# andrewdalpino/UltraZoom

Measured on AMD Instinct MI355X. Metric: upscaled MPix/sec, MewZoom-4X 1080p bf16 batched inference, higher is better.
Workload: dtype bf16; 1 GPU; MewZoom-4X 96ch/40L bf16, 16 x 1080x1920 -> 4320x7680 per GPU; global_batch=16, parallelism=batch-sharded x1, images_in_flight=0

## Files before the change

### ultrazoom_amd/csrc/mz_mix16.h

```cpp
#pragma once
#include "mz_device.h"

namespace mz {

__device__ __forceinline__ void mix_blend_pair(float& o0, float& o1, const float b0, const float b1, const float x0, const float x1,
                                               const float z0, const float z1, const float inv_s) {
    float d0, d1;
    asm("v_mul_f32 %0, 0xbfb8aa3b, %4\n\t"
        "v_mul_f32 %1, 0xbfb8aa3b, %5\n\t"
        "v_exp_f32 %0, %0\n\t"
        "v_exp_f32 %1, %1\n\t"
        "v_fma_f32 %0, %0, %10, %10\n\t"
        "v_fma_f32 %1, %1, %10, %10\n\t"
        "v_rcp_f32 %0, %0\n\t"
        "v_rcp_f32 %1, %1\n\t"
        "v_sub_f32 %2, %8, %6\n\t"
        "v_sub_f32 %3, %9, %7\n\t"
        "v_fma_f32 %0, %0, %2, %6\n\t"
        "v_fma_f32 %1, %1, %3, %7"
        : "=&v"(o0), "=&v"(o1), "=&v"(d0), "=&v"(d1)
        : "v"(b0), "v"(b1), "v"(x0), "v"(x1), "v"(z0), "v"(z1), "s"(inv_s));
}

struct MixFrag {
    u32x4 w[3][2];
};
template <class TT, int G>
__device__ __forceinline__ void mix16_group(f32x4 (&acc)[2][12], MixFrag& f, const u32x4 (&xb)[2], uint32_t b_addr) {
    constexpr int n = G % 6, wp = G % 3;
    if constexpr (G + 2 < 24) {
        f.w[(G + 2) % 3][0] = lds_read128<(((G + 2) / 6) * 12 + 2 * ((G + 2) % 6)) * 1024>(b_addr);
        f.w[(G + 2) % 3][1] = lds_read128<(((G + 2) / 6) * 12 + 2 * ((G + 2) % 6) + 1) * 1024>(b_addr);
    }
    __builtin_amdgcn_sched_barrier(0);
    constexpr int p0 = G & 1, p1 = p0 ^ 1;
    mma16<TT>(acc[p0][2 * n], f.w[wp][0], xb[p0]);
    mma16<TT>(acc[p0][2 * n + 1], f.w[wp][1], xb[p0]);
    mma16<TT>(acc[p1][2 * n + 1], f.w[wp][1], xb[p1]);
    mma16<TT>(acc[p1][2 * n], f.w[wp][0], xb[p1]);
    __builtin_amdgcn_sched_barrier(0);
    if constexpr (G + 1 < 24) wait_w16<(G + 2 < 24 ? 2 : 0)>(f.w[(G + 1) % 3][0], f.w[(G + 1) % 3][1]);
}
template <class TT, int KS> __device__ __forceinline__ void mix16_kstep(f32x4 (&acc)[2][12], MixFrag& f, const u32x4 (&xb)[2], uint32_t b_addr) {
    mix16_group<TT, KS * 6 + 0>(acc, f, xb, b_addr);
    mix16_group<TT, KS * 6 + 1>(acc, f, xb, b_addr);
    mix16_group<TT, KS * 6 + 2>(acc, f, xb, b_addr);
    mix16_group<TT, KS * 6 + 3>(acc, f, xb, b_addr);
    mix16_group<TT, KS * 6 + 4>(acc, f, xb, b_addr);
    mix16_group<TT, KS * 6 + 5>(acc, f, xb, b_addr);
}

template <class TT>
__global__ __launch_bounds__(576) void mix16_kernel(const ConvArgs a) {
    constexpr int STAGE = 4 * 12 * 1024;
    extern __shared__ __attribute__((aligned(16))) char smem[];
    const int tid = threadIdx.x;
    const int lane = tid & 63;
    const int w = __builtin_amdgcn_readfirstlane(tid >> 6);
    int mtile, ntile;
    if (!map_tile(a, mtile, ntile)) return;
    const int nsteps = a.nchunks16;
    const int nstages = nsteps >> 2;

    if (w == 8) {
        const char* src = (const char*)a.wpk16 + (size_t)ntile * nsteps * (12 * 1024) + lane * 16;
        auto issue = [&](int st) __attribute__((always_inline)) {
            char* dst = smem + (st & 1) * STAGE;
#pragma unroll
            for (int j = 0; j < 48; ++j) glds16(src + (size_t)st * STAGE + j * 1024, dst + j * 1024);
        };
        issue(0);
        for (int st = 0; st < nstages; ++st) {
            wait_vmcnt<0>();
            __builtin_amdgcn_s_barrier();
            if (st + 1 < nstages) issue(st + 1);
        }
        return;
    }

    const int g = lane >> 4, c = lane & 15;
    const long long hw = (long long)a.Ho * a.Wo;
    const long long M = (long long)a.B * hw;
    const int half_steps = nsteps >> 1;
    const uint32_t tensor_bytes = (uint32_t)((long long)a.B * a.p0 * hw * 16);
    const __amdgpu_buffer_rsrc_t xr = __builtin_amdgcn_make_buffer_rsrc((void*)a.in0, 0, (int)tensor_bytes, 0x00020000);
    const __amdgpu_buffer_rsrc_t zr = __builtin_amdgcn_make_buffer_rsrc((void*)a.in1, 0, (int)tensor_bytes, 0x00020000);
    uint32_t voff[2];
    uint32_t vpix[2];
#pragma unroll
    for (int pf = 0; pf < 2; ++pf) {
        const long long m = (long long)mtile * 256 + 32 * w + 16 * pf + c;
        const bool in = m < M;
        const long long mm = in ? m : 0;
        const int bimg = (int)(mm / hw);
        const long long pix = mm - (long long)bimg * hw;
        vpix[pf] = in ? (uint32_t)((((long long)bimg * a.p0) * hw + pix) * 16) : 0xffffffffu;
        voff[pf] = in ? (uint32_t)((((long long)bimg * a.p0 + g) * hw + pix) * 16) : 0xffffffffu;
    }
    const uint32_t step_bytes = (uint32_t)(4 * hw * 16);
    auto load_b = [&](int ks, u32x4 (&xb)[2]) __attribute__((always_inline)) {
        const bool isz = ks >= half_steps;
        const int kk = ks >= nsteps ? 0 : (isz ? ks - half_steps : ks);
        const int so = __builtin_amdgcn_readfirstlane((int)(kk * step_bytes));
#pragma unroll
        for (int pf = 0; pf < 2; ++pf)
            xb[pf] = isz ? __builtin_amdgcn_raw_buffer_load_b128(zr, (int)voff[pf], so, 0)
                         : __builtin_amdgcn_raw_buffer_load_b128(xr, (int)voff[pf], so, 0);
    };
    f32x4 acc[2][12];
#pragma unroll
    for (int pf = 0; pf < 2; ++pf)
#pragma unroll
        for (int nf = 0; nf < 12; ++nf) acc[pf][nf] = f32x4{0.f, 0.f, 0.f, 0.f};
    const uint32_t lds_base = (uint32_t)(uintptr_t)(__attribute__((address_space(3))) char*)smem;
    const uint32_t b_lane = lds_base + lane * 16;
    u32x4 xb0[2], xb1[2], xb2[2];
    load_b(0, xb0);
    load_b(1, xb1);
    MixFrag f;
    auto stage_head = [&](uint32_t b_addr) __attribute__((always_inline)) {
        __builtin_amdgcn_s_barrier();
        f.w[0][0] = lds_read128<0>(b_addr);
        f.w[0][1] = lds_read128<1024>(b_addr);
        f.w[1][0] = lds_read128<2048>(b_addr);
        f.w[1][1] = lds_read128<3072>(b_addr);
        wait_w16<2>(f.w[0][0], f.w[0][1]);
    };
    for (int st = 0; st < nstages; st += 3) {
        const int ks = 4 * st;
        uint32_t b_addr = b_lane + (st & 1) * STAGE;
        stage_head(b_addr);
        load_b(ks + 2, xb2);  mix16_kstep<TT, 0>(acc, f, xb0, b_addr);
        load_b(ks + 3, xb0);  mix16_kstep<TT, 1>(acc, f, xb1, b_addr);
        load_b(ks + 4, xb1);  mix16_kstep<TT, 2>(acc, f, xb2, b_addr);
        load_b(ks + 5, xb2);  mix16_kstep<TT, 3>(acc, f, xb0, b_addr);
        b_addr = b_lane + ((st + 1) & 1) * STAGE;
        stage_head(b_addr);
        load_b(ks + 6, xb0);  mix16_kstep<TT, 0>(acc, f, xb1, b_addr);
        load_b(ks + 7, xb1);  mix16_kstep<TT, 1>(acc, f, xb2, b_addr);
        load_b(ks + 8, xb2);  mix16_kstep<TT, 2>(acc, f, xb0, b_addr);
        load_b(ks + 9, xb0);  mix16_kstep<TT, 3>(acc, f, xb1, b_addr);
        b_addr = b_lane + (st & 1) * STAGE;
        stage_head(b_addr);
        load_b(ks + 10, xb1); mix16_kstep<TT, 0>(acc, f, xb2, b_addr);
        load_b(ks + 11, xb2); mix16_kstep<TT, 1>(acc, f, xb0, b_addr);
        load_b(ks + 12, xb0); mix16_kstep<TT, 2>(acc, f, xb1, b_addr);
        load_b(ks + 13, xb1); mix16_kstep<TT, 3>(acc, f, xb2, b_addr);
    }
    const int nbase = ntile * 192;
    const uint32_t plane_bytes = (uint32_t)(hw * 16);
    typedef uint32_t u32x2_ __attribute__((ext_vector_type(2)));
    struct XZ { u32x2_ x[2], z[2]; };
    auto request = [&](int i, XZ& q) __attribute__((always_inline)) {
        const int pf = i / 6, n = i - 6 * pf;
        const bool in = vpix[pf] != 0xffffffffu;
#pragma unroll
        for (int k = 0; k < 2; ++k) {
            const int nf = 2 * n + k;
            const int plane = (nbase >> 3) + 2 * nf + (g >> 1);
            const uint32_t off = in ? vpix[pf] + (uint32_t)plane * plane_bytes + (g & 1) * 8 : 0xffffffffu;
            q.x[k] = __builtin_amdgcn_raw_buffer_load_b64(xr, (int)off, 0, 0);
            q.z[k] = __builtin_amdgcn_raw_buffer_load_b64(zr, (int)off, 0, 0);
        }
    };
    auto finish = [&](int i, const XZ& q) __attribute__((always_inline)) {
        const int pf = i / 6, n = i - 6 * pf;
        const bool in = vpix[pf] != 0xffffffffu;
        float v[8];
#pragma unroll
        for (int k = 0; k < 2; ++k) {
            const int nf = 2 * n + k;
            float xv[4], zv[4];
            unpack2<TT>(q.x[k][0], xv[0], xv[1]); unpack2<TT>(q.x[k][1], xv[2], xv[3]);
            unpack2<TT>(q.z[k][0], zv[0], zv[1]); unpack2<TT>(q.z[k][1], zv[2], zv[3]);
            float o0, o1, o2, o3;
            mix_blend_pair(o0, o1, acc[pf][nf][0], acc[pf][nf][1], xv[0], xv[1], zv[0], zv[1], a.inv_mix_scale);
            mix_blend_pair(o2, o3, acc[pf][nf][2], acc[pf][nf][3], xv[2], xv[3], zv[2], zv[3], a.inv_mix_scale);
            acc[pf][nf] = f32x4{o0, o1, o2, o3};
        }
#pragma unroll
        for (int j = 0; j < 4; ++j) {
            const float ea = acc[pf][2 * n][j], eb = acc[pf][2 * n + 1][j];
            const auto sw = __builtin_amdgcn_permlane16_swap(__builtin_bit_cast(uint32_t, ea), __builtin_bit_cast(uint32_t, eb), false, false);
            const uint32_t s0 = sw[0], s1 = sw[1];
            v[j] = __builtin_bit_cast(float, s0);
            v[4 + j] = __builtin_bit_cast(float, s1);
        }
        const int cu = 2 * (2 * n + (g & 1)) + (g >> 1);
        if (in) st_unit<TT>((char*)a.out + vpix[pf] + (long long)((nbase >> 3) + cu) * plane_bytes, v);
    };
    XZ qa, qb;
    request(0, qa);
#pragma unroll
    for (int i = 0; i < 12; i += 2) {
        request(i + 1, qb);
        __builtin_amdgcn_sched_barrier(0);
        finish(i, qa);
        if (i + 2 < 12) request(i + 2, qa);
        __builtin_amdgcn_sched_barrier(0);
        finish(i + 1, qb);
    }
}

template <class TT>
__global__ __launch_bounds__(512) void mix16b_kernel(const ConvArgs a) {
    constexpr int STAGE = 4 * 12 * 1024;
    extern __shared__ __attribute__((aligned(16))) char smem[];
    const int tid = threadIdx.x;
    const int lane = tid & 63;
    const int w = __builtin_amdgcn_readfirstlane(tid >> 6);
    {
        const char* wsrc = (const char*)a.wpk16 + lane * 16 + w * (18 * 1024);
        char* dst = smem + w * (18 * 1024);
#pragma unroll
        for (int j = 0; j < 18; ++j) glds16(wsrc + j * 1024, dst + j * 1024);
    }
    const int g = lane >> 4, c = lane & 15;
    const long long hw = (long long)a.Ho * a.Wo;
    const long long M = (long long)a.B * hw;
    const uint32_t tensor_bytes = (uint32_t)((long long)a.B * a.p0 * hw * 16);
    const __amdgpu_buffer_rsrc_t xr = __builtin_amdgcn_make_buffer_rsrc((void*)a.in0, 0, (int)tensor_bytes, 0x00020000);
    const __amdgpu_buffer_rsrc_t zr = __builtin_amdgcn_make_buffer_rsrc((void*)a.in1, 0, (int)tensor_bytes, 0x00020000);
    const __amdgpu_buffer_rsrc_t orr = __builtin_amdgcn_make_buffer_rsrc((void*)a.out, 0, (int)tensor_bytes, 0x00020000);
    const uint32_t step_bytes = (uint32_t)(4 * hw * 16);
    const float inv_hw = 1.0f / (float)hw;
    const int hwi = (int)hw, Mi = (int)M;
    auto offsets = [&](int u, uint32_t (&vo)[2]) __attribute__((always_inline)) {
#pragma unroll
        for (int pf = 0; pf < 2; ++pf) {
            const int m = u * 32 + 16 * pf + c;
            const bool in = m < Mi;
            const int mm = in ? m : 0;
            int bimg = (int)((float)mm * inv_hw);
            int pix = mm - bimg * hwi;
            if (pix < 0) { bimg -= 1; pix += hwi; }
            if (pix >= hwi) { bimg += 1; pix -= hwi; }
            vo[pf] = in ? ((uint32_t)(bimg * a.p0 + g) * (uint32_t)hwi + (uint32_t)pix) * 16u : 0xffffffffu;
        }
    };
    const int nunits = (Mi + 31) / 32;
    const int stride = (int)gridDim.x * 8;
    int u = (int)blockIdx.x * 8 + w;
    uint32_t voff[2];
    offsets(u, voff);
    u32x4 R[12][2];
#pragma unroll
    for (int i = 0; i < 6; ++i) {
        const int so = __builtin_amdgcn_readfirstlane((int)(i * step_bytes));
#pragma unroll
        for (int pf = 0; pf < 2; ++pf) R[i][pf] = __builtin_amdgcn_raw_buffer_load_b128(xr, (int)voff[pf], so, 0);
    }
#pragma unroll
    for (int i = 0; i < 6; ++i) {
        const int so = __builtin_amdgcn_readfirstlane((int)(i * step_bytes));
#pragma unroll
        for (int pf = 0; pf < 2; ++pf) R[6 + i][pf] = __builtin_amdgcn_raw_buffer_load_b128(zr, (int)voff[pf], so, 0);
    }
    __builtin_amdgcn_sched_barrier(0);
    wait_vmcnt<0>();
    __builtin_amdgcn_s_barrier();
    const uint32_t lds_base = (uint32_t)(uintptr_t)(__attribute__((address_space(3))) char*)smem;
    const uint32_t b_lane = lds_base + lane * 16;
    MixFrag f;
    auto stage_head = [&](uint32_t b_addr) __attribute__((always_inline)) {
        f.w[0][0] = lds_read128<0>(b_addr);
        f.w[0][1] = lds_read128<1024>(b_addr);
        f.w[1][0] = lds_read128<2048>(b_addr);
        f.w[1][1] = lds_read128<3072>(b_addr);
        wait_w16<2>(f.w[0][0], f.w[0][1]);
    };
    while (u < nunits) {
        const int un = u + stride;
        uint32_t vnext[2];
        offsets(un, vnext);
        __builtin_amdgcn_sched_barrier(0);
        f32x4 acc[2][12];
#pragma unroll
        for (int pf = 0; pf < 2; ++pf)
#pragma unroll
            for (int nf = 0; nf < 12; ++nf) acc[pf][nf] = f32x4{0.f, 0.f, 0.f, 0.f};
        stage_head(b_lane);
        mix16_kstep<TT, 0>(acc, f, R[0], b_lane);
        mix16_kstep<TT, 1>(acc, f, R[1], b_lane);
        mix16_kstep<TT, 2>(acc, f, R[2], b_lane);
        mix16_kstep<TT, 3>(acc, f, R[3], b_lane);
        stage_head(b_lane + STAGE);
        mix16_kstep<TT, 0>(acc, f, R[4], b_lane + STAGE);
        mix16_kstep<TT, 1>(acc, f, R[5], b_lane + STAGE);
        mix16_kstep<TT, 2>(acc, f, R[6], b_lane + STAGE);
        mix16_kstep<TT, 3>(acc, f, R[7], b_lane + STAGE);
        stage_head(b_lane + 2 * STAGE);
        mix16_kstep<TT, 0>(acc, f, R[8], b_lane + 2 * STAGE);
        mix16_kstep<TT, 1>(acc, f, R[9], b_lane + 2 * STAGE);
        mix16_kstep<TT, 2>(acc, f, R[10], b_lane + 2 * STAGE);
        mix16_kstep<TT, 3>(acc, f, R[11], b_lane + 2 * STAGE);
#pragma unroll
        for (int m = 0; m < 6; ++m) {
            const int so = __builtin_amdgcn_readfirstlane((int)(m * step_bytes));
#pragma unroll
            for (int pf = 0; pf < 2; ++pf) {
                float v[8];
#pragma unroll
                for (int q = 0; q < 4; ++q) {
                    float xl, xh, zl, zh;
                    unpack2<TT>(R[m][pf][q], xl, xh);
                    unpack2<TT>(R[6 + m][pf][q], zl, zh);
                    mix_blend_pair(v[2 * q], v[2 * q + 1], acc[pf][2 * m + (q >> 1)][2 * (q & 1)], acc[pf][2 * m + (q >> 1)][2 * (q & 1) + 1], xl, xh, zl, zh,
                                   a.inv_mix_scale);
                }
                u32x4 t;
                if constexpr (TT::IS_BF16) {
                    t[0] = pack_bf16(v[0], v[1]); t[1] = pack_bf16(v[2], v[3]); t[2] = pack_bf16(v[4], v[5]); t[3] = pack_bf16(v[6], v[7]);
                } else {
                    t[0] = pack_f16(v[0], v[1]); t[1] = pack_f16(v[2], v[3]); t[2] = pack_f16(v[4], v[5]); t[3] = pack_f16(v[6], v[7]);
                }
                store16_soff(t, orr, (int)voff[pf], so);
            }
#pragma unroll
            for (int pf = 0; pf < 2; ++pf) {
                R[m][pf] = __builtin_amdgcn_raw_buffer_load_b128(xr, (int)vnext[pf], so, 0);
                R[6 + m][pf] = __builtin_amdgcn_raw_buffer_load_b128(zr, (int)vnext[pf], so, 0);
            }
            __builtin_amdgcn_sched_barrier(0);
        }
        u = un;
        voff[0] = vnext[0];
        voff[1] = vnext[1];
    }
}

}
```

### ultrazoom_amd/csrc/mz_mix16.hip

```cpp
#include "mz_mix16.h"

namespace mz {

hipError_t launch_mix16(int dtype, const ConvArgs& a, hipStream_t s) {
    if (!walk_ok(a)) return hipErrorInvalidValue;
    if (a.nchunks16 <= 0 || a.nchunks16 % 12) return hipErrorInvalidValue;
    const size_t lds = 2 * 4 * 12 * 1024;
    switch (dtype) {
        case DT_BF16: return launch_lds<mix16_kernel<TBF16>>(a.grid, 576, lds, a, s);
        case DT_F16: return launch_lds<mix16_kernel<TF16>>(a.grid, 576, lds, a, s);
        default: return hipErrorInvalidValue;
    }
}

hipError_t launch_mix16b(int dtype, const ConvArgs& a, hipStream_t s, int workgroups) {
    if (a.mtiles <= 0 || a.ntiles != 1 || workgroups <= 0) return hipErrorInvalidValue;
    if (a.nchunks16 != 12) return hipErrorInvalidValue;
    const size_t lds = 3 * 4 * 12 * 1024;
    const int grid = a.mtiles < workgroups ? a.mtiles : workgroups;
    switch (dtype) {
        case DT_BF16: return launch_lds<mix16b_kernel<TBF16>>(grid, 512, lds, a, s);
        case DT_F16: return launch_lds<mix16b_kernel<TF16>>(grid, 512, lds, a, s);
        default: return hipErrorInvalidValue;
    }
}

}
```

### ultrazoom_amd/csrc/mz_runner.h

```cpp
#pragma once
#include <cmath>
#include <cstring>
#include <map>
#include <utility>

#include "mz_err.h"
#include "mz_select.h"

namespace mz {

struct DevBuf {
    void* p = nullptr;
    DevBuf() = default;
    DevBuf(DevBuf&& o) noexcept : p(o.p) { o.p = nullptr; }
    ~DevBuf() {
        if (p) (void)hipFree(p);
    }
    hipError_t alloc(size_t bytes) { return p ? hipSuccess : hipMalloc(&p, bytes); }
};

struct ConvW : LayerPlan {
    DevBuf packed[PK_COUNT];
};
using BlockW = Block<ConvW>;
inline const ConvW& weights(const LayerPlan* c) { return *static_cast<const ConvW*>(c); }

inline int pack_conv(ConvW& c, int dtype, const float* w_dev, hipStream_t s) {
    for (int l = 0; l < PK_COUNT; ++l) {
        if (!c.has(l)) continue;
        HIPCHK(c.packed[l].alloc(pack_bytes(c, l)));
        HIPCHK(launch_pack(pack_args(c, l, dtype, w_dev, c.packed[l].p), s));
    }
    return MZ_OK;
}

struct ProfRec {
    hipEvent_t a, b;
    double flops, bytes;
    int kind, B, H, W, cin, cout, nt, ntiles, mtiles, n_fast;
};

struct LaunchCtx {
    DevBuf zero_page;
    Knobs knobs = read_knobs();
    std::map<std::vector<int>, std::pair<DevBuf, int>> tile_tabs;
    bool prof = false;
    std::vector<ProfRec> recs;
    size_t recs_used = 0;
    int init(hipStream_t s) {
        HIPCHK(zero_page.alloc(4096));
        HIPCHK(hipMemsetAsync(zero_page.p, 0, 4096, s));
        return MZ_OK;
    }
    ~LaunchCtx() {
        for (auto& r : recs) {
            (void)hipEventDestroy(r.a);
            (void)hipEventDestroy(r.b);
        }
    }
};

inline unsigned long long* debug_buffer() {
    static unsigned long long* buf = nullptr;
    static bool tried = false;
    if (!tried) {
        tried = true;
        if (getenv("MZ_DEBUG_STAMPS")) {
            if (hipMalloc((void**)&buf, 16 * 64 * 8 * sizeof(unsigned long long)) != hipSuccess) buf = nullptr;
            else (void)hipMemset(buf, 0, 16 * 64 * 8 * sizeof(unsigned long long));
        }
    }
    return buf;
}

inline float inv_sigmoid(float alpha) {
    const float v = 1.0f + std::exp(-alpha);
    return std::isfinite(v) ? v : 3.402823466e+38f;
}

struct Runner {
    LaunchCtx& ctx;
    hipStream_t s;
    int dtype;
    int rc = MZ_OK;
    const Knobs knobs = ctx.knobs;
    int io_u8 = 0;
    int cus = std::max(0, device_cus());

    ProfRec* prof_begin(int kind, const ConvArgs& a, const LayerPlan& c, double flops, double bytes) {
        if (!ctx.prof) return nullptr;
        if (ctx.recs_used == ctx.recs.size()) {
            ProfRec n;
            if (hipEventCreate(&n.a) != hipSuccess || hipEventCreate(&n.b) != hipSuccess) return nullptr;
            ctx.recs.push_back(n);
        }
        ProfRec* r = &ctx.recs[ctx.recs_used++];
        r->flops = flops; r->bytes = bytes;
        r->kind = kind; r->B = a.B; r->H = a.H; r->W = a.W; r->cin = c.cin; r->cout = c.cout; r->nt = c.nt; r->ntiles = a.ntiles;
        r->mtiles = a.mtiles; r->n_fast = a.gm * 1000 + a.gn;
        (void)hipEventRecord(r->a, s);
        return r;
    }

    int check(hipError_t e, const char* what) {
        if (e != hipSuccess && rc == MZ_OK) rc = hip_rc(e, what);
        return rc;
    }

    void base_args(ConvArgs& a, const ConvW& c, const void* in0, void* out, int B, int H, int W, int cp_out, const Walk& w) {
        memset(&a, 0, sizeof(a));
        a.wpk = c.packed[PK_MAIN].p;
        a.zero = ctx.zero_page.p;
        a.dbg = debug_buffer();
        a.nchunks = c.nchunks;
        a.nchunks_real = c.nchunks_real;
        a.in0 = in0; a.out = out;
        a.B = B; a.H = H; a.W = W; a.Ho = H; a.Wo = W;
        a.p0 = c.cp0 * dtype_size(dtype) / 16;
        a.cp_out = cp_out;
        a.p_out = a.cp_out * dtype_size(dtype) / 16;
        put_walk(a, w);
    }

    void tile_table(ConvArgs& a, const Walk& w, int th, int tw, int wgs) {
        const int pad = 4 * ((wgs > 256 ? wgs : 256) / 8) + 8;
        const std::vector<int> key = {th, tw, a.B, w.tiles_x, w.tiles_y, w.ntiles, w.gm, w.gn, w.grid, w.blk4, pad};
        auto it = ctx.tile_tabs.find(key);
        if (it == ctx.tile_tabs.end()) {
            std::vector<uint32_t> t;
            t.reserve(2 * ((size_t)w.mtiles * w.ntiles + pad));
            tile_list(w, th, tw, t);
            const int n = (int)(t.size() / 2);
            t.resize(t.size() + 2 * (size_t)pad, 0u);
            DevBuf d;
            if (check(d.alloc(t.size() * 4), "tile table")) return;
            if (check(hipMemcpy(d.p, t.data(), t.size() * 4, hipMemcpyHostToDevice), "tile table upload")) return;
            it = ctx.tile_tabs.emplace(key, std::make_pair(std::move(d), n)).first;
        }
        a.tile_tab = it->second.first.p;
        a.grid = it->second.second;
    }

    hipError_t launch_kernel(const KernelChoice& ch, const ConvArgs& a, int nt) {
        switch (ch.kernel) {
            case K_CONV256: return launch_conv256(dtype, ch.mode, nt, a, s);
            case K_CONV3W: return launch_conv3w(dtype, ch.mode, nt, a, s);
            case K_CONV3P: return launch_conv3p(dtype, ch.mode, nt, a, s);
            case K_CONV3S: return launch_conv3s(dtype, ch.mode, nt, a, s);
            case K_CONV3R: return launch_conv3r(dtype, a, s);
            case K_CONV3T: return launch_conv3t(dtype, a, s);
            case K_MIX16: return launch_mix16(dtype, a, s);
            case K_MIX16B: return launch_mix16b(dtype, a, s, ch.persist);
        }
        return hipErrorInvalidValue;
    }
    void launch(const KernelChoice& ch, const ConvArgs& a, int nt, ProfRec* r, const char* what = nullptr) {
        if (!what) what = g_last_kernel = kernel_name(ch);
        check(launch_kernel(ch, a, nt), what);
        if (r) (void)hipEventRecord(r->b, s);
    }

    void conv3(const Conv3Call& k) {
        if (rc) return;
        const KernelChoice ch = choose_conv3(knobs, dtype, k, cus);
        if (!ch.ok) { rc = fail(MZ_ERR_INVALID_ARGUMENT, "%s", ch.why); return; }
        const ConvW& c = weights(k.c);
        const int B = k.B, H = k.H, W = k.W;
        const double sz = dtype_size(dtype);
        const double px = (double)B * H * W;
        const int tiles_x = (W + ch.tw - 1) / ch.tw, tiles_y = (H + ch.th - 1) / ch.th;
        const Walk w = pick_order(tiles_x, tiles_y, B * tiles_x * tiles_y, c.ntiles, (double)pack_bytes(c, PK_MAIN), px * c.cp0 * sz, knobs);
        ConvArgs a;
        base_args(a, c, k.in, k.out, B, H, W, k.epi == EPI_D2S ? c.cq_p : pad16(c.cout), w);
        a.src = SRC_PLAIN;
        a.epi = k.epi; a.silu = k.silu;
        a.Hout = k.Hout; a.Wout = k.Wout;
        a.img = k.img; a.R = k.R; a.clamp = k.clamp;
        if (k.epi == EPI_FINAL) { a.Hi = k.Hout / k.R; a.Wi = k.Wout / k.R; a.io_u8 = io_u8; }
        if (k.epi == EPI_FINAL && k.views) {
            a.view = 1;
            for (int i = 0; i < 4; ++i) { a.vin[i] = k.views->in[i]; a.vout[i] = k.views->out[i]; }
            a.win_y0 = k.views->y0; a.win_x0 = k.views->x0; a.win_h = k.views->h; a.win_w = k.views->w;
        }
        const bool fused = ch.fused;
        if (fused) {
            a.in1 = k.xin;
            a.p1 = pad16(c.cout) * dtype_size(dtype) / 16;
            a.wmix = weights(k.mixf).packed[PK_MAIN].p;
            a.mix_pieces = k.mixf->nchunks * k.mixf->nt;
            const int slot = ch.mode == MODE_C3W16 ? stage_bytes<MODE_C3W16>(c.nt) : stage_bytes<MODE_C3W8>(c.nt);
            const int ncx = a.p1 / 2;
            a.x_via_lds = (a.mix_pieces * 1024 + 8 * ncx * 1024 <= 2 * slot) ? 1 : 0;
            a.mix_scale = 1.0f / (1.0f + std::exp(-k.alpha));
            a.inv_mix_scale = inv_sigmoid(k.alpha);
        }
        a.geo = ch.geo;
        a.ragged_planes = ch.ragged_planes;
        if (ch.layout != PK_MAIN) {
            a.wpk16 = c.packed[ch.layout].p;
            a.nchunks16 = pack_shape(c, ch.layout).nchunks;
            if (fused) a.wmix16 = weights(k.mixf).packed[ch.gate].p;
        }
        if (ch.tile_list) tile_table(a, w, ch.th, ch.tw, ch.persist);
        if (rc) return;
        a.persist = std::min((a.grid + 7) / 8 * 8, ch.persist);
        a.film_gamma = k.gamma; a.film_beta = k.beta;
        const double flops = 2.0 * px * 9.0 * c.cin * c.cout + (fused ? 2.0 * px * 2.0 * c.cout * c.cout : 0.0);
        const double bytes = px * (c.cin + c.cout) * sz + 9.0 * c.cin * c.cout * sz + (fused ? px * c.cout * sz : 0.0);
        launch(ch, a, c.nt, prof_begin(0, a, c, flops, bytes));
    }

    void mix(const ConvW& c, float alpha, const void* x, const void* z, void* out, int B, int H, int W) {
        if (rc) return;
        const KernelChoice ch = choose_mix(knobs, dtype, c, B, H, W, cus);
        const int sz = dtype_size(dtype);
        const long long npix = (long long)B * H * W;
        const bool mix16 = ch.layout != PK_MAIN;
        const PackShape sh = pack_shape(c, ch.layout);
        ConvArgs a;
        base_args(a, c, x, out, B, H, W, pad16(c.cout),
                  pick_order(0, 0, (int)((npix + 255) / 256), sh.ntiles, (double)pack_bytes(c, PK_MAIN),
                             (double)npix * (c.cp0 + pad16(c.c1)) * sz, knobs, mix16 ? 32 : 64));
        a.in1 = z; a.p1 = pad16(c.c1) * sz / 16;
        a.nchunks0 = c.cp0 / chunk_channels(dtype);
        a.src = SRC_CONCAT;
        a.epi = EPI_MIX;
        a.mix_scale = 1.0f / (1.0f + std::exp(-alpha));
        a.inv_mix_scale = inv_sigmoid(alpha);
        if (mix16) {
            a.wpk16 = c.packed[ch.layout].p;
            a.nchunks16 = sh.nchunks;
        }
        launch(ch, a, c.nt, prof_begin(1, a, c, 2.0 * (double)npix * c.cin * c.cout, (double)npix * 3.0 * c.cout * sz));
    }

    void crush(const ConvW& c, const void* in, void* out, int B, int H, int W) {
        if (rc) return;
        const double sz = dtype_size(dtype);
        const long long npix = (long long)B * (H / 2) * (W / 2);
        ConvArgs a;
        base_args(a, c, in, out, B, H, W, pad16(c.cout),
                  pick_order(0, 0, (int)((npix + 255) / 256), c.ntiles, (double)pack_bytes(c, PK_MAIN), (double)B * H * W * c.cp0 * sz, knobs, 64));
        a.Ho = H / 2; a.Wo = W / 2;
        a.nchunks0 = c.cp0 / chunk_channels(dtype);
        a.src = SRC_CRUSH;
        a.epi = EPI_STORE;
        ProfRec* r = prof_begin(2, a, c, 2.0 * (double)npix * 4.0 * c.cin * c.cout, ((double)B * H * W * c.cin + (double)npix * c.cout) * sz);
        KernelChoice ch;
        ch.ok = true; ch.kernel = K_CONV256; ch.mode = MODE_GEMM1;
        launch(ch, a, c.nt, r, "crush launch");
    }
};

}
```

### ultrazoom_amd/csrc/mz_select.h

```cpp
#pragma once
#include <math.h>

#include <vector>

#include "mz_plan.h"
#include "mz_view_check.h"

namespace mz {

struct Walk {
    int tiles_x = 0, tiles_y = 0;
    int mtiles = 0, ntiles = 0;
    int gm = 1, gn = 1, groups_m = 0, grid = 0;
    int blk4 = 0;
    float inv_gsz = 1.f, inv_groups_m = 1.f, inv_gn = 1.f, inv_tpi = 1.f, inv_tiles_x = 1.f, inv_bsz = 1.f;
};

inline Walk group_walk(int tiles_x, int tiles_y, int mtiles, int ntiles, int gm, int gn, int blk4) {
    Walk w;
    w.tiles_x = tiles_x; w.tiles_y = tiles_y; w.mtiles = mtiles; w.ntiles = ntiles;
    w.gm = gm; w.gn = gn; w.blk4 = blk4;
    w.groups_m = (mtiles + gm - 1) / gm;
    w.grid = (int)((long long)w.groups_m * ((ntiles + gn - 1) / gn) * gm * gn);
    w.inv_gsz = 1.0f / (float)(gm * gn);
    w.inv_groups_m = 1.0f / (float)w.groups_m;
    w.inv_gn = 1.0f / (float)gn;
    if (tiles_x > 0) {
        w.inv_tpi = 1.0f / (float)(tiles_x * tiles_y);
        w.inv_tiles_x = 1.0f / (float)tiles_x;
        w.inv_bsz = 1.0f / (float)(4 * tiles_x);
    }
    return w;
}

inline Walk pick_order(int tiles_x, int tiles_y, int mtiles, int ntiles, double weight_bytes, double act_bytes, const Knobs& k,
                       int resident_per_xcd = 32) {
    int best_gm = mtiles, best_gn = 1;
    double best = 1e300;
    for (int gn = 1; gn <= ntiles; ++gn) {
        if (gn > resident_per_xcd) break;
        if (ntiles % gn != 0 && gn != ntiles) continue;
        int gm = resident_per_xcd / gn;
        if (gm < 1) gm = 1;
        if (gm > mtiles) gm = mtiles;
        const double groups_n = ceil((double)ntiles / gn), groups_m = ceil((double)mtiles / gm);
        const double traffic = act_bytes * groups_n + weight_bytes * groups_m;
        if (traffic < best) { best = traffic; best_gm = gm; best_gn = gn; }
    }
    return group_walk(tiles_x, tiles_y, mtiles, ntiles, best_gm, best_gn, k.blk4 && tiles_x > 0 && 4 * tiles_x < 65536 ? 1 : 0);
}

inline void put_walk(ConvArgs& a, const Walk& w) {
    a.tiles_x = w.tiles_x; a.tiles_y = w.tiles_y; a.mtiles = w.mtiles; a.ntiles = w.ntiles;
    a.gm = w.gm; a.gn = w.gn; a.groups_m = w.groups_m; a.grid = w.grid; a.blk4 = w.blk4;
    a.inv_gsz = w.inv_gsz; a.inv_groups_m = w.inv_groups_m; a.inv_gn = w.inv_gn;
    a.inv_tpi = w.inv_tpi; a.inv_tiles_x = w.inv_tiles_x; a.inv_bsz = w.inv_bsz;
}

inline void tile_list(const Walk& a, int th, int tw, std::vector<uint32_t>& t) {
    const int tpi = a.tiles_x * a.tiles_y, gsz = a.gm * a.gn;
    for (int L = 0; L < a.grid; ++L) {
        const int group = L / gsz, within = L % gsz;
        const int gi_n = group / a.groups_m, gi_m = group % a.groups_m;
        const int mt = gi_m * a.gm + within / a.gn, nt = gi_n * a.gn + within % a.gn;
        if (mt >= a.mtiles || nt >= a.ntiles) continue;
        const int b = mt / tpi, trem = mt % tpi;
        int tyi, txi;
        if (!a.blk4) {
            tyi = trem / a.tiles_x; txi = trem % a.tiles_x;
        } else {
            const int bsz = 4 * a.tiles_x, br = trem / bsz, rem = trem % bsz;
            const int rows = std::min(4, a.tiles_y - 4 * br);
            txi = rem / rows; tyi = 4 * br + rem % rows;
        }
        t.push_back((uint32_t)(tyi * th) | (uint32_t)(txi * tw) << 16);
        t.push_back((uint32_t)b | (uint32_t)nt << 16);
    }
}

struct KernelChoice {
    bool ok = false;
    const char* why = nullptr;
    int kernel = K_CONV256;
    int mode = MODE_GEMM1;
    bool fused = false;
    bool mix = false;
    int th = 0, tw = 0;
    int geo = 0;
    int ragged_planes = 0;
    int layout = PK_MAIN;
    int gate = PK_MAIN;
    bool tile_list = false;
    int persist = 0;
};

inline const char* kernel_name(const KernelChoice& ch) {
    if (!ch.ok) return nullptr;
    switch (ch.kernel) {
        case K_CONV256: return ch.mix ? "conv_kernel_mix" : "conv_kernel";
        case K_CONV3W: return ch.fused ? (ch.persist > 0 ? "conv3p" : "conv3w_fused") : "conv3w";
        case K_CONV3P: return "conv3p";
        case K_CONV3S: return ch.fused ? "conv3s_fused" : "conv3s";
        case K_CONV3R: return ch.fused ? "conv3r_fused" : ch.ragged_planes ? "conv3r_ragged" : ch.geo ? "conv3r_8x40" : "conv3r";
        case K_CONV3T: return ch.fused ? "conv3t_fused" : "conv3t";
        case K_MIX16: return "mix16";
        case K_MIX16B: return "mix16b";
    }
    return nullptr;
}

inline int persistent_workgroups(const Knobs& k, int cus) { return k.persist >= 0 ? k.persist : cus; }

inline bool offsets_fit(double planes, double pixels) { return planes * pixels * 16.0 < 4294967296.0; }

struct Conv3Call {
    const LayerPlan* c = nullptr;
    const LayerPlan* mixf = nullptr;
    int epi = EPI_STORE, silu = 0;
    bool film = false;
    int B = 0, H = 0, W = 0, Hout = 0, Wout = 0;
    const void* in = nullptr;
    void* out = nullptr;
    const void* xin = nullptr;
    float alpha = 0.f;
    const void* img = nullptr;
    int R = 0, clamp = 0;
    const ImageViews* views = nullptr;
    const float *gamma = nullptr, *beta = nullptr;
};
inline Conv3Call plain_call(const LayerPlan& c, const void* in, void* out, int B, int H, int W) {
    Conv3Call k;
    k.c = &c; k.in = in; k.out = out; k.B = B; k.H = H; k.W = W;
    return k;
}
inline Conv3Call conv1_call(const LayerPlan& c, const void* in, void* out, int B, int H, int W) {
    Conv3Call k = plain_call(c, in, out, B, H, W);
    k.silu = 1;
    return k;
}
inline Conv3Call d2s_call(const LayerPlan& c, const void* in, void* out, int B, int H, int W, int Hout, int Wout) {
    Conv3Call k = plain_call(c, in, out, B, H, W);
    k.epi = EPI_D2S; k.Hout = Hout; k.Wout = Wout;
    return k;
}
inline Conv3Call head_call(const LayerPlan& c, const void* in, void* out, int B, int H, int W) {
    Conv3Call k = plain_call(c, in, out, B, H, W);
    k.epi = EPI_FINAL; k.Hout = 2 * H; k.Wout = 2 * W;
    return k;
}
inline Conv3Call film_call(const LayerPlan& c, const void* in, void* out, int B, int H, int W, int silu) {
    Conv3Call k = plain_call(c, in, out, B, H, W);
    k.film = true; k.silu = silu;
    return k;
}
template <class Layer> Conv3Call fused_call(const Block<Layer>& b, const void* in, const void* xin, void* out, int B, int H, int W) {
    Conv3Call k = plain_call(b.conv2, in, out, B, H, W);
    k.epi = EPI_FUSEDMIX; k.mixf = &b.mixf; k.xin = xin; k.alpha = b.alpha;
    return k;
}
template <class Layer> Conv3Call conv2_call(const Knobs& k, const Block<Layer>& b, const void* in, const void* xin, int B, int H, int W) {
    return b.fused && k.wide && k.fuse ? fused_call(b, in, xin, nullptr, B, H, W) : plain_call(b.conv2, in, nullptr, B, H, W);
}

inline KernelChoice choose_conv3(const Knobs& k, int dtype, const Conv3Call& call, int cus) {
    KernelChoice ch;
    const LayerPlan& c = *call.c;
    const LayerPlan* mixf = call.mixf;
    const int epi = call.epi, B = call.B, H = call.H, W = call.W;
    const bool fused = epi == EPI_FUSEDMIX;
    const int wgs = persistent_workgroups(k, cus);
    const double px = (double)H * W;
    int mode = MODE_CONV3, th = 8, tw = 32;
    if (c.nt <= 3 && k.wide) {
        const long long waste16 = (long long)((H + 15) / 16 * 16) * ((W + 31) / 32 * 32);
        const long long waste8 = (long long)((H + 7) / 8 * 8) * ((W + 63) / 64 * 64);
        if (waste8 <= waste16) { mode = MODE_C3W8; th = 8; tw = 64; }
        else { mode = MODE_C3W16; th = 16; tw = 32; }
    }
    if (epi == EPI_FINAL && dtype != DT_F32) { mode = MODE_CONV3; th = 8; tw = 32; }
    ch.mode = mode;

    const bool s16 = k.s16 && dtype != DT_F32 && wgs > 0;
    const bool k_fits = c.nchunks32 * 32 * 100 <= c.cp0 * (100 + k.kpad_pct);
    const bool halo_fits = offsets_fit(4, px);
    const int p0 = c.cp0 * dtype_size(dtype) / 16;
    auto listed = [&](int kernel, int lth, int ltw, int layout, int gate) {
        ch.kernel = kernel; ch.fused = fused; ch.th = lth; ch.tw = ltw;
        ch.layout = layout; ch.gate = gate;
        ch.tile_list = true;
        ch.persist = wgs;
        ch.ok = B < 65536 && c.ntiles < 65536 && (H + lth - 1) / lth * lth < 65536 && (W + ltw - 1) / ltw * ltw < 65536;
        if (!ch.ok) ch.why = "tile table: image, batch or N-tile index beyond 16 bits";
        return ch;
    };

    const bool t_fuse = epi == EPI_FUSEDMIX && k.fuse16 && mixf && mixf->has(PK_GATE16T);
    if (k.t && s16 && !call.film && c.has(PK_CONV16T) && c.ntiles == 1 && (c.nchunks32 == 3 || c.nchunks32 >= 6) &&
        (epi == EPI_STORE || t_fuse) && halo_fits && offsets_fit(6, px))
        return listed(K_CONV3T, 12, 64, PK_CONV16T, t_fuse ? PK_GATE16T : PK_MAIN);

    if (k.r && k.r2 && s16 && !call.film && c.nt == 3 && c.has(PK_CONV16) && epi == EPI_STORE && call.silu && c.nchunks32 == 2 && c.cp0 == 48 &&
        halo_fits && offsets_fit(12, px)) {
        ch.ragged_planes = (c.cp0 - 32) / 8;
        return listed(K_CONV3R, 8, 48, PK_CONV16, PK_MAIN);
    }

    if (k.r && k.fuse16 && epi == EPI_FUSEDMIX && s16 && c.nt == 3 && c.ntiles == 1 && c.has(PK_CONV16) && mixf && mixf->has(PK_GATE16R) &&
        mixf->nchunks32 == c.nt && c.nchunks32 >= 6 && p0 % 4 == 0 && k_fits && halo_fits && offsets_fit(12, px))
        return listed(K_CONV3R, 8, 48, PK_CONV16, PK_GATE16R);

    if (k.r && s16 && !call.film && c.nt == 3 && c.has(PK_CONV16) && (epi == EPI_STORE || epi == EPI_D2S) && k_fits && halo_fits &&
        c.nchunks32 >= 3 && p0 % 4 == 0 &&
        (epi == EPI_D2S ? offsets_fit(c.cq_p * dtype_size(dtype) / 16, (double)call.Hout * call.Wout) : offsets_fit(12, px))) {
        const long long rows8 = (long long)((H + 7) / 8 * 8);
        const long long pad48 = rows8 * ((W + 47) / 48 * 48), pad40 = rows8 * ((W + 39) / 40 * 40);
        const long long pads = (long long)((H + th - 1) / th) * th * ((W + tw - 1) / tw) * tw;
        const int geo = pad40 < pad48 ? 1 : 0;
        if ((geo ? pad40 : pad48) <= pads) {
            ch.geo = geo;
            return listed(K_CONV3R, 8, geo ? 40 : 48, PK_CONV16, PK_MAIN);
        }
    }

    ch.th = th; ch.tw = tw;
    ch.fused = fused;
    const bool fuse16 = fused && mixf && mixf->has(PK_GATE16) && k.fuse16 &&
                        mixf->nchunks32 == c.nt;
    if (mode != MODE_CONV3 && (epi == EPI_STORE || epi == EPI_D2S || fuse16) && wgs > 0) {
        const int tiles_x = (W + tw - 1) / tw, tiles_y = (H + th - 1) / th;
        const Walk g = pick_order(tiles_x, tiles_y, B * tiles_x * tiles_y, c.ntiles, (double)pack_bytes(c, PK_MAIN),
                                  (double)B * H * W * c.cp0 * (double)dtype_size(dtype), k);
        if (s16 && c.has(PK_CONV16) && k_fits && halo_fits) {
            ch.layout = PK_CONV16;
            ch.gate = fused ? PK_GATE16 : PK_MAIN;
            ch.persist = wgs;
        } else if (g.grid > wgs && offsets_fit(2, px)) {
            ch.persist = wgs;
        }
    }
    if (call.film && ch.layout == PK_MAIN) {
        ch.why = "the FiLM epilogue exists on the 16x16x32 kernel only: bf16 / fp16, at most 96 output channels per "
                 "N tile, input channels within 12.5 % of a multiple of 32";
        return ch;
    }
    ch.kernel = mode == MODE_CONV3 ? K_CONV256 : ch.persist == 0 || (fused && ch.layout == PK_MAIN) ? K_CONV3W : ch.layout != PK_MAIN ? K_CONV3S : K_CONV3P;
    ch.ok = true;
    return ch;
}

inline KernelChoice choose_mix(const Knobs& k, int dtype, const LayerPlan& c, int B, int H, int W, int cus) {
    KernelChoice ch;
    ch.ok = ch.mix = true;
    ch.mode = MODE_GEMM1;
    const bool mix16 = c.has(PK_MIX16) && offsets_fit(c.cp0 * dtype_size(dtype) / 16.0, (double)B * H * W);
    const int wgs = k.persist > 0 ? k.persist : cus;
    if (mix16 && k.mix16b && c.has(PK_MIX16B) && wgs > 0) {
        ch.kernel = K_MIX16B; ch.layout = PK_MIX16B; ch.persist = wgs;
    } else if (mix16) {
        ch.kernel = K_MIX16; ch.layout = PK_MIX16;
    } else {
        ch.kernel = K_CONV256;
    }
    return ch;
}

inline const LayerPlan* plan_debug_layer(BlockPlan& b, int dtype, int op, int cin, int cout, Refusal* why) {
    switch (op) {
        case 0: case 1: case 2: case 3: case 4: case 5:
            plan_conv(b.conv1, dtype, MODE_CONV3, cout, cin, 3, 3, op == 2 ? OUT_D2S : op == 3 ? OUT_FINAL : OUT_PLAIN, SRC_PLAIN, 0, 0);
            return &b.conv1;
        case 6: case 8:
            plan_block(b, dtype, cout, cin);
            if (op == 6) return &b.conv2;
            if (b.fused) return &b.mixf;
            *why = refuse(MZ_ERR_INVALID_ARGUMENT, "the block does not fuse conv2 and the mix");
            return nullptr;
        case 7:
            if (cin == 2 * cout) {
                plan_conv(b.mix, dtype, MODE_GEMM1, cout, cin, 1, 1, OUT_PLAIN, SRC_CONCAT, cout, cout);
                return &b.mix;
            }
            *why = refuse(MZ_ERR_INVALID_ARGUMENT, "a mix has cin = 2 cout");
            return nullptr;
    }
    *why = refuse(MZ_ERR_INVALID_ARGUMENT, "bad op %d", op);
    return nullptr;
}

}
```

Before: 704.3 MPix/s.

## Make mix16 kernel persistent with XCD-aware tile walk and cross-tile prefetch

```diff
diff --git a/ultrazoom_amd/csrc/mz_mix16.h b/ultrazoom_amd/csrc/mz_mix16.h
--- a/ultrazoom_amd/csrc/mz_mix16.h
+++ b/ultrazoom_amd/csrc/mz_mix16.h
@@ -57,66 +57,99 @@
     const int tid = threadIdx.x;
     const int lane = tid & 63;
     const int w = __builtin_amdgcn_readfirstlane(tid >> 6);
-    int mtile, ntile;
-    if (!map_tile(a, mtile, ntile)) return;
+    const int xcd = blockIdx.x & 7, pos = blockIdx.x >> 3;
+    const int q = a.grid >> 3, rem = a.grid & 7;
+    const int cnt = q + (xcd < rem ? 1 : 0);
+    const int base = xcd < rem ? xcd * (q + 1) : rem * (q + 1) + (xcd - rem) * q;
+    const int step = a.persist > 0 ? (int)(gridDim.x >> 3) : cnt;
+    auto seek = [&](int i, int& mt, int& nt) __attribute__((always_inline)) {
+        while (i < cnt && !tile_of(a, base + i, mt, nt)) i += step;
+        return i;
+    };
+    int mtile = 0, ntile = 0;
+    int cur = seek(pos, mtile, ntile);
+    if (cur >= cnt) return;
     const int nsteps = a.nchunks16;
     const int nstages = nsteps >> 2;
 
     if (w == 8) {
-        const char* src = (const char*)a.wpk16 + (size_t)ntile * nsteps * (12 * 1024) + lane * 16;
-        auto issue = [&](int st) __attribute__((always_inline)) {
-            char* dst = smem + (st & 1) * STAGE;
+        auto wsrc = [&](int nt) __attribute__((always_inline)) { return (const char*)a.wpk16 + (size_t)nt * nsteps * (12 * 1024) + lane * 16; };
+        auto issue = [&](const char* src, int st, int slot) __attribute__((always_inline)) {
+            char* dst = smem + (slot & 1) * STAGE;
 #pragma unroll
             for (int j = 0; j < 48; ++j) glds16(src + (size_t)st * STAGE + j * 1024, dst + j * 1024);
         };
-        issue(0);
-        for (int st = 0; st < nstages; ++st) {
-            wait_vmcnt<0>();
-            __builtin_amdgcn_s_barrier();
-            if (st + 1 < nstages) issue(st + 1);
-        }
-        return;
-    }
-
-    const int g = lane >> 4, c = lane & 15;
-    const long long hw = (long long)a.Ho * a.Wo;
-    const long long M = (long long)a.B * hw;
-    const int half_steps = nsteps >> 1;
-    const uint32_t tensor_bytes = (uint32_t)((long long)a.B * a.p0 * hw * 16);
+        const char* src = wsrc(ntile);
+        int par = 0;
+        issue(src, 0, 0);
+        for (;;) {
+            int mt_n = 0, nt_n = 0;
+            const int nxt = seek(cur + step, mt_n, nt_n);
+            const bool more = nxt < cnt;
+            const char* src_n = wsrc(nt_n);
+            for (int st = 0; st < nstages; ++st) {
+                wait_vmcnt<0>();
+                __builtin_amdgcn_s_barrier();
+                if (st + 1 < nstages) issue(src, st + 1, par + st + 1);
+                else if (more) issue(src_n, 0, par + nstages);
+            }
+            if (!more) return;
+            par = (par + nstages) & 1;
+            src = src_n;
+            cur = nxt;
+        }
+    }
+
+    const int hwi = a.Ho * a.Wo, Mi = a.B * hwi;
+    const float inv_hw = __builtin_bit_cast(float, __builtin_amdgcn_readfirstlane(__builtin_bit_cast(int, 1.0f / (float)hwi)));
+    auto lane_gc = [&](int& g, int& c) __attribute__((always_inline)) {
+        int ln = lane;
+        asm volatile("" : "+v"(ln));
+        g = ln >> 4; c = ln & 15;
+    };
+    const uint32_t tensor_bytes = (uint32_t)Mi * (uint32_t)a.p0 * 16u;
     const __amdgpu_buffer_rsrc_t xr = __builtin_amdgcn_make_buffer_rsrc((void*)a.in0, 0, (int)tensor_bytes, 0x00020000);
     const __amdgpu_buffer_rsrc_t zr = __builtin_amdgcn_make_buffer_rsrc((void*)a.in1, 0, (int)tensor_bytes, 0x00020000);
+    const uint32_t plane_bytes = (uint32_t)hwi * 16u;
+    const uint32_t step_bytes = 4 * plane_bytes;
     uint32_t voff[2];
+    uint32_t voffn[2];
     uint32_t vpix[2];
-#pragma unroll
-    for (int pf = 0; pf < 2; ++pf) {
-        const long long m = (long long)mtile * 256 + 32 * w + 16 * pf + c;
-        const bool in = m < M;
-        const long long mm = in ? m : 0;
-        const int bimg = (int)(mm / hw);
-        const long long pix = mm - (long long)bimg * hw;
-        vpix[pf] = in ? (uint32_t)((((long long)bimg * a.p0) * hw + pix) * 16) : 0xffffffffu;
-        voff[pf] = in ? (uint32_t)((((long long)bimg * a.p0 + g) * hw + pix) * 16) : 0xffffffffu;
-    }
-    const uint32_t step_bytes = (uint32_t)(4 * hw * 16);
-    auto load_b = [&](int ks, u32x4 (&xb)[2]) __attribute__((always_inline)) {
-        const bool isz = ks >= half_steps;
-        const int kk = ks >= nsteps ? 0 : (isz ? ks - half_steps : ks);
-        const int so = __builtin_amdgcn_readfirstlane((int)(kk * step_bytes));
-#pragma unroll
-        for (int pf = 0; pf < 2; ++pf)
-            xb[pf] = isz ? __builtin_amdgcn_raw_buffer_load_b128(zr, (int)voff[pf], so, 0)
-                         : __builtin_amdgcn_raw_buffer_load_b128(xr, (int)voff[pf], so, 0);
-    };
-    f32x4 acc[2][12];
-#pragma unroll
-    for (int pf = 0; pf < 2; ++pf)
-#pragma unroll
-        for (int nf = 0; nf < 12; ++nf) acc[pf][nf] = f32x4{0.f, 0.f, 0.f, 0.f};
+    auto offsets = [&](uint32_t (&vo)[2], int mt, bool real, int g, int c) __attribute__((always_inline)) {
+#pragma unroll
+        for (int pf = 0; pf < 2; ++pf) {
+            const int m = mt * 256 + 32 * w + 16 * pf + c;
+            const bool in = real && m < Mi;
+            const int mm = in ? m : 0;
+            int bimg = (int)((float)mm * inv_hw);
+            int pix = mm - bimg * hwi;
+            if (pix < 0) { bimg -= 1; pix += hwi; }
+            if (pix >= hwi) { bimg += 1; pix -= hwi; }
+            vo[pf] = in ? ((uint32_t)(bimg * a.p0 + g) * (uint32_t)hwi + (uint32_t)pix) * 16u : 0xffffffffu;
+        }
+    };
+    const int half_steps = nsteps >> 1;
+    auto load_b = [&](int ks, u32x4 (&xb)[2], bool tail = false) __attribute__((always_inline)) {
+        const bool past = tail && ks >= nsteps;
+        const int k = past ? ks - nsteps : ks;
+        const bool isz = k >= half_steps;
+        const int so = __builtin_amdgcn_readfirstlane((int)((isz ? k - half_steps : k) * step_bytes));
+        const __amdgpu_buffer_rsrc_t r = isz ? zr : xr;
+#pragma unroll
+        for (int pf = 0; pf < 2; ++pf) {
+            u32x4& dst = xb[pf];
+            const uint32_t vo = past ? voffn[pf] : voff[pf];
+            asm volatile("buffer_load_dwordx4 %0, %1, %2, %3 offen" : "+v"(dst) : "v"(vo), "s"(r), "s"(so) : "memory");
+        }
+    };
+    auto landed = [&](u32x4 (&xb)[2], bool wait) __attribute__((always_inline)) {
+        u32x4 &x0 = xb[0], &x1 = xb[1];
+        if (wait) wait_vmcnt<4>();
+        asm volatile("" : "+v"(x0), "+v"(x1)::"memory");
+    };
     const uint32_t lds_base = (uint32_t)(uintptr_t)(__attribute__((address_space(3))) char*)smem;
     const uint32_t b_lane = lds_base + lane * 16;
-    u32x4 xb0[2], xb1[2], xb2[2];
-    load_b(0, xb0);
-    load_b(1, xb1);
+    u32x4 xb0[2] = {}, xb1[2] = {}, xb2[2] = {};
     MixFrag f;
     auto stage_head = [&](uint32_t b_addr) __attribute__((always_inline)) {
         __builtin_amdgcn_s_barrier();
@@ -126,32 +159,11 @@
         f.w[1][1] = lds_read128<3072>(b_addr);
         wait_w16<2>(f.w[0][0], f.w[0][1]);
     };
-    for (int st = 0; st < nstages; st += 3) {
-        const int ks = 4 * st;
-        uint32_t b_addr = b_lane + (st & 1) * STAGE;
-        stage_head(b_addr);
-        load_b(ks + 2, xb2);  mix16_kstep<TT, 0>(acc, f, xb0, b_addr);
-        load_b(ks + 3, xb0);  mix16_kstep<TT, 1>(acc, f, xb1, b_addr);
-        load_b(ks + 4, xb1);  mix16_kstep<TT, 2>(acc, f, xb2, b_addr);
-        load_b(ks + 5, xb2);  mix16_kstep<TT, 3>(acc, f, xb0, b_addr);
-        b_addr = b_lane + ((st + 1) & 1) * STAGE;
-        stage_head(b_addr);
-        load_b(ks + 6, xb0);  mix16_kstep<TT, 0>(acc, f, xb1, b_addr);
-        load_b(ks + 7, xb1);  mix16_kstep<TT, 1>(acc, f, xb2, b_addr);
-        load_b(ks + 8, xb2);  mix16_kstep<TT, 2>(acc, f, xb0, b_addr);
-        load_b(ks + 9, xb0);  mix16_kstep<TT, 3>(acc, f, xb1, b_addr);
-        b_addr = b_lane + (st & 1) * STAGE;
-        stage_head(b_addr);
-        load_b(ks + 10, xb1); mix16_kstep<TT, 0>(acc, f, xb2, b_addr);
-        load_b(ks + 11, xb2); mix16_kstep<TT, 1>(acc, f, xb0, b_addr);
-        load_b(ks + 12, xb0); mix16_kstep<TT, 2>(acc, f, xb1, b_addr);
-        load_b(ks + 13, xb1); mix16_kstep<TT, 3>(acc, f, xb2, b_addr);
-    }
-    const int nbase = ntile * 192;
-    const uint32_t plane_bytes = (uint32_t)(hw * 16);
+    f32x4 acc[2][12];
+    int nbase = 0;
     typedef uint32_t u32x2_ __attribute__((ext_vector_type(2)));
     struct XZ { u32x2_ x[2], z[2]; };
-    auto request = [&](int i, XZ& q) __attribute__((always_inline)) {
+    auto request = [&](int i, XZ& q, int g) __attribute__((always_inline)) {
         const int pf = i / 6, n = i - 6 * pf;
         const bool in = vpix[pf] != 0xffffffffu;
 #pragma unroll
@@ -163,7 +175,7 @@
             q.z[k] = __builtin_amdgcn_raw_buffer_load_b64(zr, (int)off, 0, 0);
         }
     };
-    auto finish = [&](int i, const XZ& q) __attribute__((always_inline)) {
+    auto finish = [&](int i, const XZ& q, int g) __attribute__((always_inline)) {
         const int pf = i / 6, n = i - 6 * pf;
         const bool in = vpix[pf] != 0xffffffffu;
         float v[8];
@@ -189,16 +201,71 @@
         const int cu = 2 * (2 * n + (g & 1)) + (g >> 1);
         if (in) st_unit<TT>((char*)a.out + vpix[pf] + (long long)((nbase >> 3) + cu) * plane_bytes, v);
     };
-    XZ qa, qb;
-    request(0, qa);
-#pragma unroll
-    for (int i = 0; i < 12; i += 2) {
-        request(i + 1, qb);
-        __builtin_amdgcn_sched_barrier(0);
-        finish(i, qa);
-        if (i + 2 < 12) request(i + 2, qa);
-        __builtin_amdgcn_sched_barrier(0);
-        finish(i + 1, qb);
+
+    int mtile_n = 0, ntile_n = 0;
+    int nxt = seek(cur + step, mtile_n, ntile_n);
+    {
+        int g, c;
+        lane_gc(g, c);
+        offsets(voff, mtile, true, g, c);
+        offsets(voffn, mtile_n, nxt < cnt, g, c);
+    }
+    load_b(0, xb0);
+    load_b(1, xb1);
+    wait_vmcnt<0>();
+    int par = 0;
+    for (;;) {
+#pragma unroll
+        for (int pf = 0; pf < 2; ++pf)
+#pragma unroll
+            for (int nf = 0; nf < 12; ++nf) acc[pf][nf] = f32x4{0.f, 0.f, 0.f, 0.f};
+        for (int st = 0; st < nstages; st += 3) {
+            const int ks = 4 * st;
+            const uint32_t b_even = b_lane + ((par + st) & 1) * STAGE, b_odd = b_lane + ((par + st + 1) & 1) * STAGE;
+            stage_head(b_even);
+            load_b(ks + 2, xb2);  landed(xb0, st != 0); mix16_kstep<TT, 0>(acc, f, xb0, b_even);
+            load_b(ks + 3, xb0);  landed(xb1, st != 0); mix16_kstep<TT, 1>(acc, f, xb1, b_even);
+            load_b(ks + 4, xb1);  landed(xb2, true);    mix16_kstep<TT, 2>(acc, f, xb2, b_even);
+            load_b(ks + 5, xb2);  landed(xb0, true);    mix16_kstep<TT, 3>(acc, f, xb0, b_even);
+            stage_head(b_odd);
+            load_b(ks + 6, xb0);  landed(xb1, true);    mix16_kstep<TT, 0>(acc, f, xb1, b_odd);
+            load_b(ks + 7, xb1);  landed(xb2, true);    mix16_kstep<TT, 1>(acc, f, xb2, b_odd);
+            load_b(ks + 8, xb2);  landed(xb0, true);    mix16_kstep<TT, 2>(acc, f, xb0, b_odd);
+            load_b(ks + 9, xb0);  landed(xb1, true);    mix16_kstep<TT, 3>(acc, f, xb1, b_odd);
+            stage_head(b_even);
+            load_b(ks + 10, xb1); landed(xb2, true);    mix16_kstep<TT, 0>(acc, f, xb2, b_even);
+            load_b(ks + 11, xb2); landed(xb0, true);    mix16_kstep<TT, 1>(acc, f, xb0, b_even);
+            load_b(ks + 12, xb0, true); landed(xb1, true);    mix16_kstep<TT, 2>(acc, f, xb1, b_even);
+            load_b(ks + 13, xb1, true); landed(xb2, true);    mix16_kstep<TT, 3>(acc, f, xb2, b_even);
+        }
+        par = (par + nstages) & 1;
+        int g, c;
+        lane_gc(g, c);
+#pragma unroll
+        for (int pf = 0; pf < 2; ++pf) {
+            vpix[pf] = voff[pf] != 0xffffffffu ? voff[pf] - (uint32_t)g * plane_bytes : 0xffffffffu;
+            voff[pf] = voffn[pf];
+        }
+        nbase = ntile * 192;
+        const bool more = nxt < cnt;
+        if (more) {
+            cur = nxt; mtile = mtile_n; ntile = ntile_n;
+            nxt = seek(cur + step, mtile_n, ntile_n);
+        }
+        offsets(voffn, mtile_n, more && nxt < cnt, g, c);
+        XZ qa, qb;
+        request(0, qa, g);
+#pragma unroll
+        for (int i = 0; i < 12; i += 2) {
+            request(i + 1, qb, g);
+            __builtin_amdgcn_sched_barrier(0);
+            finish(i, qa, g);
+            if (i + 2 < 12) request(i + 2, qa, g);
+            __builtin_amdgcn_sched_barrier(0);
+            finish(i + 1, qb, g);
+        }
+        if (!more) return;
+        wait_vmcnt<48>();
     }
 }
 
diff --git a/ultrazoom_amd/csrc/mz_mix16.hip b/ultrazoom_amd/csrc/mz_mix16.hip
--- a/ultrazoom_amd/csrc/mz_mix16.hip
+++ b/ultrazoom_amd/csrc/mz_mix16.hip
@@ -5,10 +5,12 @@
 hipError_t launch_mix16(int dtype, const ConvArgs& a, hipStream_t s) {
     if (!walk_ok(a)) return hipErrorInvalidValue;
     if (a.nchunks16 <= 0 || a.nchunks16 % 12) return hipErrorInvalidValue;
+    if (a.persist < 0 || (a.persist & 7)) return hipErrorInvalidValue;
     const size_t lds = 2 * 4 * 12 * 1024;
+    const int grid = a.persist > 0 ? a.persist : a.grid;
     switch (dtype) {
-        case DT_BF16: return launch_lds<mix16_kernel<TBF16>>(a.grid, 576, lds, a, s);
-        case DT_F16: return launch_lds<mix16_kernel<TF16>>(a.grid, 576, lds, a, s);
+        case DT_BF16: return launch_lds<mix16_kernel<TBF16>>(grid, 576, lds, a, s);
+        case DT_F16: return launch_lds<mix16_kernel<TF16>>(grid, 576, lds, a, s);
         default: return hipErrorInvalidValue;
     }
 }
diff --git a/ultrazoom_amd/csrc/mz_runner.h b/ultrazoom_amd/csrc/mz_runner.h
--- a/ultrazoom_amd/csrc/mz_runner.h
+++ b/ultrazoom_amd/csrc/mz_runner.h
@@ -231,6 +231,7 @@
             a.wpk16 = c.packed[ch.layout].p;
             a.nchunks16 = sh.nchunks;
         }
+        if (ch.kernel == K_MIX16) a.persist = std::min((a.grid + 7) / 8 * 8, ch.persist);
         launch(ch, a, c.nt, prof_begin(1, a, c, 2.0 * (double)npix * c.cin * c.cout, (double)npix * 3.0 * c.cout * sz));
     }
 
diff --git a/ultrazoom_amd/csrc/mz_select.h b/ultrazoom_amd/csrc/mz_select.h
--- a/ultrazoom_amd/csrc/mz_select.h
+++ b/ultrazoom_amd/csrc/mz_select.h
@@ -257,7 +257,7 @@
     if (mix16 && k.mix16b && c.has(PK_MIX16B) && wgs > 0) {
         ch.kernel = K_MIX16B; ch.layout = PK_MIX16B; ch.persist = wgs;
     } else if (mix16) {
-        ch.kernel = K_MIX16; ch.layout = PK_MIX16;
+        ch.kernel = K_MIX16; ch.layout = PK_MIX16; ch.persist = persistent_workgroups(k, cus) / 8 * 8;
     } else {
         ch.kernel = K_CONV256;
     }
```

Measured after the change: 704.8 MPix/s (median of 2 runs). No clear change (+0.1%).
